# gildas-lormeau/zlib-streams-ts

Measured on AMD Instinct MI355X. Metric: uncompressed MB/s, deflate-raw L6, 4096x64KiB batch at 1/2/4/8 GPUs, higher is better.
Workload: dtype u8; 1 GPU; 4096 x 65536 B text-corpus streams split across the GPUs, deflate-raw level 6; global_streams=4096, streams_per_gpu=4096, stream_bytes=65536, level=6, format=deflate-raw, compressed_bytes=91855591, parallelism=dp1

## Files before the change

zlib-streams-ts_amd/csrc/capi.cpp:

```cpp
#include <hip/hip_runtime.h>
#include <stdint.h>
#include <stdio.h>
#include <string.h>

#include <algorithm>
#include <string>
#include <thread>
#include <type_traits>
#include <vector>

#include "../../include/zs_gpu.h"
#include "zs_common.h"
#include "zs_kernels.h"
#include "zs_inflate.h"
#include "zs_split.h"
#include "zs_seg.h"
#include "zs_plan.h"
#include "zs_dict.h"


namespace {

thread_local std::string g_err;

int fail(int code, const char* fmt, const char* a = "") {
  char buf[512];
  snprintf(buf, sizeof buf, fmt, a);
  g_err = buf;
  return code;
}

#define HIPCHK(x)                                                          \
  do {                                                                     \
    hipError_t e_ = (x);                                                   \
    if (e_ != hipSuccess) return fail(ZS_MEM_ERROR, "%s", hipGetErrorString(e_)); \
  } while (0)

template <bool kHost>
struct BufT {
  void* p = nullptr;
  size_t cap = 0;
  BufT() = default;
  BufT(const BufT&) = delete;
  BufT& operator=(const BufT&) = delete;
  ~BufT() { release(); }
  void release() {
    if (p) (void)(kHost ? hipHostFree(p) : hipFree(p));
    p = nullptr;
    cap = 0;
  }
// ... 384 lines not shown
  HIPCHK(hipGetLastError());
  return ZS_OK;
}

struct DeflDict {
  const Batch* data;
  const uint32_t *start, *did, *dadler;
};
static int deflate_launch(zs_ctx* c, hipStream_t st, int level, int wrap, const zs_level_cfg& cfg, const Batch& b,
                          const MetaLayout& ml, int32_t* d_status, uint32_t* d_out_len, const DeflDict* dd = nullptr) {
  const zs_deflate_plan& p = c->dp;
  const uint32_t n = b.n;
  const uint8_t* dm = c->meta.as<uint8_t>();
  const uint64_t* d_pos = (const uint64_t*)(dm + ml.pos_base);
  const uint32_t* d_blk = (const uint32_t*)(dm + ml.blk_base);
  const zs_sweep_seg* d_segs = (const zs_sweep_seg*)(dm + ml.segs);
  zs_stream* d_st = c->streams.as<zs_stream>();
  zs_block* d_bk = c->blocks.as<zs_block>();
  uint32_t* syms = c->syms.as<uint32_t>();
  uint32_t* check = c->check.as<uint32_t>();
  const int nthreads_s = 256, nblocks_s = (int)((n + 255) / 256);
  MARK("start");
  if (wrap) {
    const Batch& d = dd ? *dd->data : b;
    zs_k_checksum<<<n, 64, 0, st>>>(d.in, d.in_off, d.in_len, check, wrap == 1 ? 1 : 2);
    zs_k_copy_check<<<nblocks_s, nthreads_s, 0, st>>>(check, d_st, (int)n);
    MARK("checksum");
  }
  if (level >= 4 && c->o.match_sweep) {
    const uint32_t nw = (uint32_t)p.segs.size();
    (c->lane_order ? zs_k_bucket<true> : zs_k_bucket<false>)<<<nw, ZS_BK_THREADS, 0, st>>>(
        b.in, b.in_off, b.in_len, d_pos, d_segs, c->prevd.as<uint16_t>(), c->mres.as<uint2>());
    MARK("bucket");
    zs_k_sweep<<<nw, 1024, 0, st>>>(b.in, b.in_off, b.in_len, d_pos, d_segs, c->prevd.as<uint16_t>(),
                                    c->mres.as<uint2>(), cfg.chain, cfg.nice);
    MARK("sweep");
  } else if (level >= 4) {
    const dim3 g((p.max_len + 8191) / 8192, n);
    (c->lane_order ? zs_k_prev<true> : zs_k_prev<false>)<<<n, 64, 0, st>>>(b.in, b.in_off, b.in_len, d_pos,
                                                                           c->prevd.as<uint16_t>(), 0u);
    MARK("prev");
    if (p.max_len) zs_k_match<<<g, 1024, 0, st>>>(b.in, b.in_off, b.in_len, d_pos, c->prevd.as<uint16_t>(),
                                                   c->mres.as<uint2>(), cfg.chain, cfg.nice, 0u);
    MARK("match");
  }
  if (level >= 4) {
    const int pw = p.pw;
    if (dd) {
      auto parse = pw == 4 ? zs_k_parse_4w_dict : pw == 2 ? zs_k_parse_2w_dict : zs_k_parse_dict;
      parse<<<n, 64 * pw, 0, st>>>(b.in, b.in_off, b.in_len, d_pos, d_blk, c->mres.as<uint2>(), syms, d_bk, d_st,
                                   c->pscr.as<uint32_t>(), cfg.good, cfg.lazy, dd->start);
    } else {
      auto parse = pw == 4 ? zs_k_parse_4w : pw == 2 ? zs_k_parse_2w : zs_k_parse;
      parse<<<n, 64 * pw, 0, st>>>(b.in, b.in_off, b.in_len, d_pos, d_blk, c->mres.as<uint2>(), syms, d_bk, d_st,
                                   c->pscr.as<uint32_t>(), cfg.good, cfg.lazy);
    }
    MARK("parse");
  } else {
    const int fast_smem = 2 * 32768 * 2 + 32768;
    auto pick = [&](auto D) {
      constexpr bool DICT = decltype(D)::value;
      return !c->fast_group ? zs_k_fast_serial<DICT>
             : c->lane_order ? (cfg.nice <= 8 ? zs_k_fast<2, true, DICT> : cfg.nice <= 16 ? zs_k_fast<4, true, DICT> : zs_k_fast<8, true, DICT>)
                             : (cfg.nice <= 8 ? zs_k_fast<2, false, DICT> : cfg.nice <= 16 ? zs_k_fast<4, false, DICT> : zs_k_fast<8, false, DICT>);
    };
    auto fast = dd ? pick(std::true_type{}) : pick(std::false_type{});
    HIPCHK(hipFuncSetAttribute((const void*)fast, hipFuncAttributeMaxDynamicSharedMemorySize, fast_smem));
    fast<<<n, 64, fast_smem, st>>>(b.in, b.in_off, b.in_len, d_pos, d_blk, syms, d_bk, d_st, cfg.chain, cfg.lazy,
// ... 990 lines not shown
```

zlib-streams-ts_amd/csrc/deflate_sweep.hip:

```cpp
#include <hip/hip_runtime.h>
#include "zs_common.h"
#include "zs_kernels.h"
#include "zs_sweep_ring.h"
#include "zs_sweep_long.h"
#include <type_traits>

#define ZS_SW_WIN_WORDS ((ZS_SEG_WPOS + 258u + 20u + 3u) / 4u + 2u)
#define ZS_SW_RING 128u
#define ZS_SW_MW 320u
#ifndef ZS_SW_RUN_CAP
#define ZS_SW_RUN_CAP 16u
#endif

typedef __attribute__((address_space(3))) uint32_t zs_sw_lds_u32;
static __device__ __forceinline__ uint32_t sw_lds_addr(const void* p) {
  return (uint32_t)(uintptr_t)(const zs_sw_lds_u32*)p;
}

static __device__ __forceinline__ uint32_t sw_hash(uint32_t w) {
  return (((w & 0xffu) << 10) ^ (((w >> 8) & 0xffu) << 5) ^ ((w >> 16) & 0xffu)) & ZS_HASH_MASK;
}

#define ZS_BK_WPT (16384u / ZS_BK_THREADS)
#define ZS_BK_PPL (ZS_BK_THREADS / 64u)
#ifndef ZS_BK_PROF
#define ZS_BK_PROF 0
#endif
#if ZS_BK_PROF
__device__ unsigned long long zs_bk_stat[4];
extern "C" int zs_bucket_stats(unsigned long long* out) {
  return (int)hipMemcpyFromSymbol(out, HIP_SYMBOL(zs_bk_stat), sizeof(zs_bk_stat));
}
#define BK_MARK(i) do { if (threadIdx.x == 0) { const unsigned long long t_ = wall_clock64(); atomicAdd(&zs_bk_stat[i], t_ - bk_t); bk_t = t_; } } while (0)
#else
#define BK_MARK(i) do { } while (0)
#endif
#define ZS_BK_INFLIGHT 8
#define ZS_BK_CHUNK 2048u
// ... 163 lines not shown
          if (p < c1) qc[p - c0] = (uint16_t)(e[j] >> sh[j]);
        }
      }
    } else if (wave != 0 && c > 0) {
      const uint32_t b0 = c0 - ZS_BK_CHUNK, cnt1 = min(m, c0) - b0;
      const uint16_t* const qp = q[(c - 1) & 1u];
      for (uint32_t o = tid - 64u; o < cnt1; o += ZS_BK_THREADS - 64u) mem[qp[o]] = (uint16_t)(b0 + o);
    }
    __syncthreads();
  }
  BK_MARK(2);
}
template __global__ void zs_k_bucket<true>(const uint8_t*, const uint64_t*, const uint32_t*, const uint64_t*,
                                           const zs_sweep_seg*, uint16_t*, uint2*);
template __global__ void zs_k_bucket<false>(const uint8_t*, const uint64_t*, const uint32_t*, const uint64_t*,
                                            const zs_sweep_seg*, uint16_t*, uint2*);

static __device__ __forceinline__ uint32_t sw_word(const uint32_t* win, uint32_t off) {
  const uint32_t i = off >> 2;
  return __builtin_amdgcn_alignbyte(win[i + 1], win[i], off & 3u);
}

static __device__ __forceinline__ uint32_t sw_extend(const uint32_t* win, uint32_t p, uint32_t q, uint32_t maxc,
                                                     uint32_t from) {
  uint32_t k = from;
  while (k < maxc) {
    const uint32_t y = sw_word(win, q + k) ^ sw_word(win, p + k);
    if (y) { k += (uint32_t)(__builtin_ctz(y) >> 3); break; }
    k += 4;
  }
  return k < maxc ? k : maxc;
}

static __device__ __forceinline__ uint64_t sw_uniform(uint64_t x) {
  return ((uint64_t)(uint32_t)__builtin_amdgcn_readfirstlane((uint32_t)(x >> 32)) << 32) |
         (uint64_t)(uint32_t)__builtin_amdgcn_readfirstlane((uint32_t)x);
}

static __device__ __forceinline__ uint32_t max3(uint32_t a, uint32_t b, uint32_t c) {
  return max(max(a, b), c);
}

static __device__ __forceinline__ uint32_t sw_x7(uint32_t w) {
  const uint32_t b0 = w & 0xffu, b1 = (w >> 8) & 0xffu;
  return ((b0 >> 5) & 3u) | ((b1 & 7u) << 2) | (((b1 >> 5) & 3u) << 5);
}
template <bool A7>
struct SwSig;
template <>
struct SwSig<false> {
  static constexpr uint32_t LONG = 88u;
  static constexpr uint32_t THR0 = 23u;
  static constexpr uint32_t EXT = 11u;
  uint32_t a, b, c;
  static __device__ __forceinline__ uint4 rec(const uint32_t* win, uint32_t q, uint32_t w0) {
    return make_uint4(w0, sw_word(win, q + 4), sw_word(win, q + 8) & 0x00ffffffu, 0u);
  }
  __device__ __forceinline__ uint32_t mbits(uint32_t x, uint32_t y, uint32_t z) const {
    uint32_t f0, f1, f2;
    asm("v_ffbl_b32 %0, %1" : "=v"(f0) : "v"(x ^ a));
    asm("v_ffbl_b32 %0, %1\n\tv_add_u32_e64 %0, %0, 32 clamp" : "=&v"(f1) : "v"(y ^ b));
    asm("v_ffbl_b32 %0, %1\n\tv_add_u32_e32 %0, 64, %0" : "=&v"(f2) : "v"(z ^ c));
    return min(min(f0, f1), f2);
  }
  static __device__ __forceinline__ uint32_t len(uint32_t sigma) { return sigma; }
};
template <>
struct SwSig<true> {
  static constexpr uint32_t LONG = 64u;
  static constexpr uint32_t THR0 = 7u;
  static constexpr uint32_t EXT = 10u;
  uint32_t a, b;
  static __device__ __forceinline__ uint4 rec(const uint32_t* win, uint32_t q, uint32_t w0) {
    return make_uint4(sw_x7(w0) | (sw_word(win, q + 3) << 8), sw_word(win, q + 6), sw_word(win, q + EXT), 0u);
  }
  __device__ __forceinline__ uint32_t mbits(uint32_t x, uint32_t y, uint32_t) const {
    uint32_t f0, f1;
    asm("v_ffbl_b32 %0, %1" : "=v"(f0) : "v"(x ^ a));
    asm("v_ffbl_b32 %0, %1\n\tv_add_u32_e64 %0, %0, 32 clamp" : "=&v"(f1) : "v"(y ^ b));
    return min(min(f0, f1), 64u);
  }
  static __device__ __forceinline__ uint32_t len(uint32_t sigma) { return sigma ? sigma + 2u : 2u; }
};

struct SwRing {
  uint2 ab[2 * ZS_SW_RING];
  uint32_t c[2 * ZS_SW_RING];
  uint32_t key[2 * ZS_SW_RING];
  __device__ __forceinline__ void put(int b, uint32_t lane, uint4 r) {
    const uint32_t i = (uint32_t)(64 * b + (int)lane) & (ZS_SW_RING - 1);
    ab[i] = make_uint2(r.x, r.y);
    ab[i + ZS_SW_RING] = make_uint2(r.x, r.y);
    c[i] = r.z;
    c[i + ZS_SW_RING] = r.z;
    key[i] = r.w;
    key[i + ZS_SW_RING] = r.w;
  }
  static __device__ __forceinline__ uint32_t base(int c, uint32_t s, uint32_t lane) {
    return ((uint32_t)(64 * (c - (int)s - 1) + (int)lane) & (ZS_SW_RING - 1)) + 64u * s + 64u;
  }
};
struct SwRingP {
  uint2 ab[ZS_SWR_SLOTS + ZS_SWR_MIRROR];
  uint32_t c[ZS_SWR_SLOTS + ZS_SWR_MIRROR];
  uint32_t key[ZS_SWR_SLOTS + ZS_SWR_MIRROR];
  __device__ __forceinline__ void put(int b, uint32_t lane, uint4 r) {
    const uint32_t i = zs_swr_block_slot(b) + lane;
    ab[i] = make_uint2(r.x, r.y);
    c[i] = r.z;
    key[i] = r.w;
    if (zs_swr_mirrored(b)) {
      ab[i + ZS_SWR_SLOTS] = make_uint2(r.x, r.y);
      c[i + ZS_SWR_SLOTS] = r.z;
      key[i + ZS_SWR_SLOTS] = r.w;
    }
  }
  static __device__ __forceinline__ uint32_t base(int c, uint32_t s, uint32_t lane) { return zs_swr_base(c, s) + lane; }
  __device__ __forceinline__ uint32_t pos(int c, uint32_t lane, uint32_t t) const {
    return key[zs_swr_member_slot(c, lane, t)] & 0xffffu;
  }
};

#ifndef ZS_SW_PROF
#define ZS_SW_PROF 0
#endif
#if ZS_SW_PROF
__device__ unsigned long long zs_sw_stat[8];
#define SW_STAT(i, v) do { if ((threadIdx.x & 63u) == __builtin_ctzll(__builtin_amdgcn_read_exec())) atomicAdd(&zs_sw_stat[i], (unsigned long long)(v)); } while (0)
extern "C" int zs_sw_stats(unsigned long long* out) {
  return (int)hipMemcpyFromSymbol(out, HIP_SYMBOL(zs_sw_stat), sizeof(zs_sw_stat));
}
#else
#define SW_STAT(i, v) do { } while (0)
#endif

static __device__ __forceinline__ uint32_t sw_score(uint32_t mb, uint32_t u) { return (mb & ~7u) | (7u - u); }
template <uint32_t N>
static __device__ __forceinline__ uint32_t sw_gmax(const uint32_t* sc) {
  static_assert(N == 8 || N == 4 || N == 3 || N == 1, "group sizes");
  if constexpr (N == 8) return max(max3(sc[0], sc[1], sc[2]), max3(sc[3], sc[4], max3(sc[5], sc[6], sc[7])));
  else if constexpr (N == 4) return max3(sc[0], sc[1], max(sc[2], sc[3]));
  else if constexpr (N == 3) return max3(sc[0], sc[1], sc[2]);
  else return sc[0];
}

template <bool A7>
struct SwLane {
  SwSig<A7> S;
  uint32_t p;
  bool own;
  uint32_t maxc, nice;
  uint32_t khead, klim;
  uint32_t long_m;
  uint32_t own_ext;
  uint32_t thr, bt, thr_s, bt_s;
  uint32_t lthr, lbt, lthr_s, lbt_s;
  uint64_t alive_m;
  uint32_t head;
  bool snapped;
  __device__ __forceinline__ bool tail() const { return maxc <= 12u; }
  __device__ __forceinline__ void snap() {
    thr_s = thr;
    bt_s = bt;
    lthr_s = lthr;
    lbt_s = lbt;
    snapped = true;
  }
};

template <bool A7, bool MW, bool PR>
struct SwWave {
  using Sig = SwSig<A7>;
  using Lane = SwLane<A7>;
  using Ring = std::conditional_t<PR, SwRingP, SwRing>;
  const uint32_t* win;
  Ring* R;
  uint16_t* mw;
  const uint16_t* mem;
  uint32_t n, m, lane;
  uint32_t budget, budget_s, nice_cfg;
  int cc;
  zs_swr_range vr;
  int mw0;

  __device__ __forceinline__ int k() const { return 64 * cc + (int)lane; }
  __device__ __forceinline__ uint32_t fetch(int j) const { return j >= 0 && (uint32_t)j < m ? (uint32_t)mem[j] : 0u; }
  __device__ __forceinline__ uint4 make_rec(uint32_t q) const {
    const uint32_t w0 = sw_word(win, q);
    uint4 r = Sig::rec(win, q, w0);
    r.w = (sw_hash(w0) << 16) | q;
    return r;
  }
  __device__ __forceinline__ void build_blk(int blk, uint32_t q) {
    const int j = 64 * blk + (int)lane;
    const bool in = j >= 0 && (uint32_t)j < m;
    if (MW && (uint32_t)(j - mw0) < ZS_SW_MW) mw[j - mw0] = (uint16_t)q;
    R->put(blk, lane, in ? make_rec(q) : make_uint4(0, 0, 0, 0));
    if constexpr (PR) vr = zs_swr_extend(vr, blk);
  }
  __device__ __forceinline__ bool missing(int blk) const { return !PR || !zs_swr_has(vr, blk); }
  __device__ __forceinline__ uint32_t member(uint32_t t) const {
    if constexpr (PR) return R->pos(cc, lane, t);
    const int j = k() - (int)t;
// ... 9 lines not shown
    L.p = p;
    L.own = own;
    const uint32_t h = rown.w >> 16;
    const uint32_t look = n - p;
    L.maxc = look < ZS_MAX_MATCH ? look : ZS_MAX_MATCH;
    L.nice = look < nice_cfg ? look : nice_cfg;
    L.long_m = L.tail() ? 0xffffu : Sig::LONG;
    const uint32_t limit = p > ZS_MAX_DIST ? p - ZS_MAX_DIST : 0u;
    L.khead = (h << 16) | (limit > 1u ? limit : 1u);
    L.klim = (h << 16) | limit;
    L.thr = L.thr_s = Sig::THR0;
    L.bt = L.bt_s = 0;
    L.lthr = L.lthr_s = ZS_SWL_NONE;
    L.lbt = L.lbt_s = 0;
    L.alive_m = 0;
    L.head = 0;
    L.snapped = budget_s <= 1u;
    return rown;
  }

  __device__ __forceinline__ void build(uint4 rown, uint32_t p, uint32_t qb, bool have_qb) {
    mw0 = 64 * cc - (int)budget;
    if (MW) mw[k() - mw0] = (uint16_t)p;
    __builtin_amdgcn_s_waitcnt(0xc07f);
    __builtin_amdgcn_wave_barrier();
    R->put(cc, lane, rown);
    if constexpr (PR) vr = zs_swr_push(vr, cc);
    if (missing(cc - 1)) build_blk(cc - 1, have_qb ? qb : fetch(k() - 64));
    __builtin_amdgcn_s_waitcnt(0xc07f);
    __builtin_amdgcn_wave_barrier();
  }

  __device__ __forceinline__ void fold(Lane& L, uint32_t gm, uint32_t t0, const uint32_t* sc, uint32_t cnt,
                                       uint32_t base) const {
    const bool up = gm > (L.thr | 7u);
    L.thr = up ? gm : L.thr;
    L.bt = up ? t0 : L.bt;
    if (__builtin_expect(__builtin_amdgcn_ballot_w64(gm >= L.long_m) != 0, 0)) {
      SW_STAT(3, 1);
      auto lscore = [&](uint32_t u) -> uint32_t {
        const uint32_t ls = base - (t0 + u);
        const uint32_t x = (A7 ? R->c[ls] : sw_word(win, (R->key[ls] & 0xffffu) + Sig::EXT)) ^ L.own_ext;
        const uint32_t len = x ? Sig::EXT + ((uint32_t)__builtin_ctz(x) >> 3)
                               : sw_extend(win, L.p, R->key[ls] & 0xffffu, L.maxc, Sig::EXT + 4u);
        return zs_swl_score(len, L.maxc, L.nice, u);
      };
      const bool lg = gm >= L.long_m && zs_swl_open(L.lthr, L.nice);
      uint32_t w[2] = {0, 0};
#pragma unroll
      for (uint32_t u = 0; u < 8; u++)
        if (u < cnt) w[u >> 2] |= sc[u] << (8u * (u & 3u));
      constexpr uint32_t LB = (0x80u - Sig::LONG) * 0x01010101u;
      const uint32_t nl = (uint32_t)__builtin_popcount((w[0] + LB) & 0x80808080u) +
                          (uint32_t)__builtin_popcount((w[1] + LB) & 0x80808080u);
      const uint64_t twice = __builtin_amdgcn_ballot_w64(lg && nl > 1u);
      uint32_t gl = 0;
      const uint32_t u1 = zs_swl_first(gm);
      if (lg) gl = lscore(u1);
      if (__builtin_expect(twice != 0, 0)) {
        if ((twice >> lane) & 1u) {
          uint32_t lm = 0;
#pragma unroll
          for (uint32_t u = 0; u < 8; u++) lm |= (u < cnt && sc[u] >= L.long_m) ? 1u << u : 0u;
          lm &= ~(1u << u1);
          while (lm) {
            gl = zs_swl_join(gl, lscore((uint32_t)__builtin_ctz(lm)));
            lm &= lm - 1u;
          }
        }
      }
      zs_swl_fold(gl, t0, &L.lthr, &L.lbt);
    }
  }

  template <uint32_t N>
  __device__ __forceinline__ void group_fast(Lane& L, uint32_t base, uint32_t t0, bool live) const {
    const uint32_t lo = base - (t0 + (N - 1u));
    const uint2* const A = R->ab + lo;
    const uint32_t* const C = R->c + lo;
    uint32_t sc[N];
#pragma unroll
    for (uint32_t u = 0; u < N; u++) {
      const uint2 ab = A[N - 1u - u];
      sc[u] = sw_score(L.S.mbits(ab.x, ab.y, A7 ? 0u : C[N - 1u - u]), u);
    }
    fold(L, live ? sw_gmax<N>(sc) : 0u, t0, sc, N, base);
  }
  template <uint32_t N, bool HEAD>
  __device__ __forceinline__ void group_masked(Lane& L, uint32_t base, uint32_t t0) const {
    const uint32_t lo = base - (t0 + (N - 1u));
    const uint2* const A = R->ab + lo;
    const uint32_t* const C = R->c + lo;
    const uint32_t* const K = R->key + lo;
    uint32_t sc[N], key[N];
    uint2 ab[N];
#pragma unroll
    for (uint32_t u = 0; u < N; u++) {
      key[u] = K[N - 1u - u];
      ab[u] = A[N - 1u - u];
    }
    if constexpr (HEAD) {
      const bool a1 = L.own && key[0] >= L.khead;
      L.head = a1 ? 1u | ((L.p - (key[0] & 0xffffu)) == ZS_MAX_DIST ? 0x8000u : 0u) : 0u;
      L.alive_m = __builtin_amdgcn_ballot_w64(a1);
    }
    uint64_t lm = L.alive_m;
#pragma unroll
    for (uint32_t u = 0; u < N; u++) {
      if (!HEAD || u) {
        asm("v_cmp_gt_u32_e64 %0, %1, %2" : "=s"(lm) : "v"(key[u]), "v"(L.klim));
        lm &= L.alive_m;
      }
      const uint32_t v = sw_score(L.S.mbits(ab[u].x, ab[u].y, A7 ? 0u : C[N - 1u - u]), u);
      asm("v_cndmask_b32_e64 %0, 0, %1, %2" : "=v"(sc[u]) : "v"(v), "s"(lm));
    }
    L.alive_m = sw_uniform(lm);
    fold(L, sw_gmax<N>(sc), t0, sc, N, base);
  }

  __device__ __forceinline__ void run(Lane& L, uint32_t base, uint32_t ta, uint32_t tb) const {
    auto last_of = [&](uint32_t t0) __attribute__((always_inline)) {
      uint32_t t1 = t0 + 7u <= tb ? t0 + 7u : t0 + 3u;
      if (t0 <= budget_s && t1 > budget_s) t1 = budget_s;
      return t1;
    };
    if (ta > tb) return;
    uint32_t t0 = ta, t1 = last_of(ta);
    uint32_t kl = R->key[base - t1];
    while (L.alive_m) {
      const bool mine = ((L.alive_m >> lane) & 1u) != 0;
      const uint64_t last_live = __builtin_amdgcn_ballot_w64(mine && kl > L.klim);
      const uint32_t n0 = t1 + 1u, n1 = n0 <= tb ? last_of(n0) : t1;
      kl = R->key[base - n1];
      SW_STAT(last_live == L.alive_m ? 1 : 2, 1);
      SW_STAT(4, t1 - t0 + 1u);
      if (last_live == L.alive_m) {
        if (t1 - t0 == 7u) group_fast<8>(L, base, t0, mine);
        else group_fast<4>(L, base, t0, mine);
      } else {
        if (t1 - t0 == 7u) group_masked<8, false>(L, base, t0);
        else group_masked<4, false>(L, base, t0);
      }
      if (t1 == budget_s) L.snap();
      if (n0 > tb) break;
      t0 = n0;
      t1 = n1;
    }
  }

  __device__ __forceinline__ void sweep(Lane& L) {
    const uint32_t base0 = Ring::base(cc, 0u, lane);
    const bool open8 = budget_s >= 8u && budget >= 8u;
    if (open8) {
      group_masked<8, true>(L, base0, 1u);
      if (budget_s == 8u) L.snap();
    } else {
      group_masked<1, true>(L, base0, 1u);
      if (budget_s == 1u) L.snap();
      if (budget >= 4u) {
        group_masked<3, false>(L, base0, 2u);
        if (budget_s == 4u) L.snap();
      }
    }
    for (uint32_t b = 0; budget > 4u && L.alive_m; b++) {
      const int blk = cc - (int)b - 1;
      if (b >= 1 && missing(blk)) {
        __builtin_amdgcn_s_waitcnt(0xc07f);
        __builtin_amdgcn_wave_barrier();
        build_blk(blk, fetch(64 * blk + (int)lane));
        __builtin_amdgcn_s_waitcnt(0xc07f);
        __builtin_amdgcn_wave_barrier();
      }
      const uint32_t ta = b == 0 ? (open8 ? 9u : 5u) : 64u * b + 1u;
      const uint32_t tb = min(64u * b + 64u, budget);
      run(L, Ring::base(cc, b, lane), ta, tb);
      if (tb >= budget) break;
    }
    if (!L.snapped) L.snap();
  }

  __device__ __forceinline__ void settle(const Lane& L, uint2* out) const {
    __builtin_amdgcn_s_waitcnt(0xc07f);
    __builtin_amdgcn_wave_barrier();
    if (!L.own) return;
    const uint32_t p = L.p;
    uint32_t rx = 0, ry = 0;
    if (L.head) {
      uint32_t len = 2, dist = 0, len_s = 2, dist_s = 0;
      if (L.tail()) {
        const int k = this->k();
        uint32_t b = 2u << 16, bs = 2u << 16;
        for (uint32_t t = 1; t <= budget && (int)t <= k; t++) {
          const uint32_t q = member(t);
          const uint32_t key = (sw_hash(sw_word(win, q)) << 16) | q;
          if (t == 1u ? key < L.khead : key <= L.klim) break;
          uint32_t len = 12;
          for (uint32_t o = 0; o < 12u; o += 4) {
            const uint32_t y = sw_word(win, q + o) ^ sw_word(win, p + o);
            if (y) { len = o + (uint32_t)(__builtin_ctz(y) >> 3); break; }
          }
          const uint32_t sc = ((len < L.maxc ? len : L.maxc) << 16) | (0xffffu - t);
          b = max(b, sc);
          if (t <= budget_s) bs = max(bs, sc);
        }
        len = b >> 16;
        dist = len > 2u ? p - (uint32_t)mem[k - (int)(0xffffu - (b & 0xffffu))] : 0u;
        len_s = bs >> 16;
        dist_s = len_s > 2u ? p - (uint32_t)mem[k - (int)(0xffffu - (bs & 0xffffu))] : 0u;
      } else {
        const uint32_t tb = L.bt + 7u - (L.thr & 7u), tb_s = L.bt_s + 7u - (L.thr_s & 7u);
        if (L.bt) {
          len = Sig::len(L.thr >> 3);
          dist = p - member(tb);
        }
        if (L.bt_s) {
          len_s = Sig::len(L.thr_s >> 3);
          dist_s = tb_s == tb ? dist : p - member(tb_s);
        }
        auto long_of = [&](uint32_t lt, uint32_t t, uint32_t& ln, uint32_t& ds) {
          const uint32_t q = member(t);
          ln = lt >> 3;
          if (ln >= L.nice) ln = sw_extend(win, p, q, L.maxc, Sig::EXT);
          ds = p - q;
        };
        if (L.lbt) long_of(L.lthr, L.lbt, len, dist);
        if (L.lbt_s) {
          if (L.lbt_s == L.lbt) {
            len_s = len;
            dist_s = dist;
          } else {
            long_of(L.lthr_s, L.lbt_s, len_s, dist_s);
          }
        }
      }
      rx = (len << 16) | (len > 2u ? dist : 0u) | (L.head & 0x8000u);
      ry = (len_s << 16) | (len_s > 2u ? dist_s : 0u);
    }
    out[p] = make_uint2(rx, ry);
  }
};

template <bool A7, bool MW, bool PR>
static __device__ __forceinline__ void sw_body(const uint32_t* win, void* ringp, uint16_t* mw, uint32_t* next,
                                               uint32_t n, uint32_t m, uint32_t olo, uint32_t ohi,
                                               const uint16_t* mem, uint2* out, int chain, int nice_cfg) {
  using Wave = SwWave<A7, MW, PR>;
  const uint32_t lane = threadIdx.x & 63u;
  Wave W{win, (typename Wave::Ring*)ringp, mw, mem, n, m, lane, (uint32_t)chain, (uint32_t)chain >> 2,
         (uint32_t)nice_cfg, 0, zs_swr_empty(), 0};
  const uint32_t nchunks = (m + 63) / 64;
  auto claim = [&]() -> uint32_t {
    uint32_t c = 0;
    if (lane == 0) c = atomicAdd(next, 1u);
    return __builtin_amdgcn_readfirstlane(c);
  };
  auto claim_run = [&](uint32_t& c0, uint32_t& c1) {
    uint32_t a = 0, r = 0;
    if (lane == 0) {
      const uint32_t cur = __hip_atomic_load(next, __ATOMIC_RELAXED, __HIP_MEMORY_SCOPE_WORKGROUP);
      r = zs_swr_run_len(cur < nchunks ? nchunks - cur : 0u, ZS_SW_RUN_CAP);
      a = atomicAdd(next, r);
    }
    c0 = __builtin_amdgcn_readfirstlane(a);
    c1 = min(c0 + (uint32_t)__builtin_amdgcn_readfirstlane(r), nchunks);
  };
  uint32_t c, ce = 0;
  if constexpr (PR) claim_run(c, ce);
  else c = claim();
  uint32_t pf_p = W.fetch((int)(64 * c + lane)), pf_b = W.fetch((int)(64 * c + lane) - 64);
  bool fresh_n = true;
  for (;;) {
    if (c >= nchunks) break;
    const bool fresh = fresh_n;
    uint32_t cn, cen = ce;
    if constexpr (PR) {
      cn = c + 1u;
      fresh_n = cn >= ce;
      if (fresh_n) claim_run(cn, cen);
      if (fresh) W.vr = zs_swr_empty();
    } else {
      cn = claim();
    }
    W.cc = (int)c;
    const bool mem_ok = (uint32_t)W.k() < m;
    SW_STAT(0, 1);
    const uint32_t p = pf_p, qb = pf_b;
    if (cn < nchunks) {
      pf_p = W.fetch((int)(64 * cn + lane));
      if (!PR || fresh_n) pf_b = W.fetch((int)(64 * cn + lane) - 64);
    }
    c = cn;
    ce = cen;
    const bool own = mem_ok && p >= olo && p < ohi;
    if (__builtin_amdgcn_ballot_w64(own) == 0) {
      W.vr = zs_swr_empty();
      continue;
    }
    typename Wave::Lane L;
    const uint4 rown = W.start(L, p, mem_ok, own);
    W.build(rown, p, qb, fresh);
    W.sweep(L);
    W.settle(L, out);
  }
}

__global__ __launch_bounds__(1024) void zs_k_sweep(const uint8_t* __restrict__ in, const uint64_t* __restrict__ in_off,
                                                   const uint32_t* __restrict__ in_len,
                                                   const uint64_t* __restrict__ pos_base,
                                                   const zs_sweep_seg* __restrict__ segs,
                                                   const uint16_t* __restrict__ members, uint2* __restrict__ mres,
                                                   int chain, int nice_cfg) {
  constexpr uint32_t RING_BYTES = 16u * sizeof(SwRing), MWIN_BYTES = 16u * ZS_SW_MW * sizeof(uint16_t);
  static_assert(16u * sizeof(SwRingP) <= RING_BYTES + MWIN_BYTES, "the persistent rings must fit the old ones' LDS");
  __shared__ __attribute__((aligned(16))) uint8_t rmem[RING_BYTES + MWIN_BYTES];
  __shared__ __attribute__((aligned(16))) uint32_t win[ZS_SW_WIN_WORDS];
  __shared__ uint32_t next;
  const zs_sweep_seg G = segs[blockIdx.x];
  const int s = (int)G.s;
  const uint32_t n = in_len[s] - G.base;
  if (n < 3) return;
  const uint32_t m = min(n - 2, G.ohi);
  const uint8_t* src = in + in_off[s] + G.base;
  uint32_t hi = 0;
  if ((((uintptr_t)src) & 15u) == 0) {
    for (uint32_t i = threadIdx.x; 4 * i < ZS_SW_WIN_WORDS; i += 1024) {
      const uint32_t b = 16 * i;
      uint4 v;
      if (b + 16 <= n) v = ((const uint4*)src)[i];
      else {
        uint32_t t[4] = {0, 0, 0, 0};
        for (uint32_t k = 0; k < 16; k++)
          if (b + k < n) t[k >> 2] |= (uint32_t)src[b + k] << (8 * (k & 3));
        v = make_uint4(t[0], t[1], t[2], t[3]);
      }
      hi |= v.x | v.y | v.z | v.w;
      if (4 * i + 3 < ZS_SW_WIN_WORDS) *(uint4*)(win + 4 * i) = v;
      else for (uint32_t k = 0; 4 * i + k < ZS_SW_WIN_WORDS; k++) win[4 * i + k] = (&v.x)[k];
    }
  } else {
    for (uint32_t i = threadIdx.x; i < ZS_SW_WIN_WORDS; i += 1024) {
      uint32_t v = 0;
      for (uint32_t k = 0; k < 4; k++)
        if (4 * i + k < n) v |= (uint32_t)src[4 * i + k] << (8 * k);
      hi |= v;
      win[i] = v;
    }
  }
  if (threadIdx.x == 0) next = 0;
  const bool a7 = !__syncthreads_or((hi & 0x80808080u) != 0);
  const uint32_t wave = threadIdx.x >> 6;
  const uint16_t* mem = members + G.mb;
  uint2* out = mres + pos_base[s] + G.base;
  const uint32_t olo = G.olo, ohi = G.ohi;
  if (chain <= (int)ZS_SWR_MAX_CHAIN) {
    SwRingP* const R = reinterpret_cast<SwRingP*>(rmem) + wave;
    if (a7) sw_body<true, false, true>(win, R, nullptr, &next, n, m, olo, ohi, mem, out, chain, nice_cfg);
    else sw_body<false, false, true>(win, R, nullptr, &next, n, m, olo, ohi, mem, out, chain, nice_cfg);
    return;
  }
  SwRing* const R = reinterpret_cast<SwRing*>(rmem) + wave;
  uint16_t* const mw = reinterpret_cast<uint16_t*>(rmem + RING_BYTES) + wave * ZS_SW_MW;
  if (chain + 64 <= (int)ZS_SW_MW) {
    if (a7) sw_body<true, true, false>(win, R, mw, &next, n, m, olo, ohi, mem, out, chain, nice_cfg);
    else sw_body<false, true, false>(win, R, mw, &next, n, m, olo, ohi, mem, out, chain, nice_cfg);
  } else {
    if (a7) sw_body<true, false, false>(win, R, mw, &next, n, m, olo, ohi, mem, out, chain, nice_cfg);
    else sw_body<false, false, false>(win, R, mw, &next, n, m, olo, ohi, mem, out, chain, nice_cfg);
  }
}
```

zlib-streams-ts_amd/csrc/zs_kernels.h:

```cpp
#pragma once
#include <hip/hip_runtime.h>
#include <stdint.h>
#include "zs_plan.h"

struct zs_block {
  uint32_t sym_start;
  uint32_t sym_count;
  uint32_t in_start;
  uint32_t in_end;
  uint32_t type;
  uint32_t hdr_bits;
  uint32_t data_bits;
  uint32_t last;
  uint32_t pad;
  uint64_t bit_off;
  uint64_t bit_end;
};

struct zs_stream {
  uint32_t nsym;
  uint32_t nblk;
  uint64_t total_bits;
  uint32_t out_len;
  int32_t status;
  uint32_t check;
  uint32_t pad;
};

template <bool ORD>
__global__ void zs_k_prev(const uint8_t* in, const uint64_t* in_off, const uint32_t* in_len, const uint64_t* pos_base,
                          uint16_t* prevd, uint32_t min_len);
__global__ void zs_k_match(const uint8_t* in, const uint64_t* in_off, const uint32_t* in_len, const uint64_t* pos_base,
                           const uint16_t* prevd, uint2* mres, int chain, int nice, uint32_t min_len);
#define ZS_BK_THREADS 512u
template <bool ORD>
__global__ void zs_k_bucket(const uint8_t* in, const uint64_t* in_off, const uint32_t* in_len, const uint64_t* pos_base,
                            const zs_sweep_seg* segs, uint16_t* members, uint2* mres);
__global__ void zs_k_sweep(const uint8_t* in, const uint64_t* in_off, const uint32_t* in_len, const uint64_t* pos_base,
                           const zs_sweep_seg* segs, const uint16_t* members, uint2* mres, int chain, int nice);
#define ZS_PARSE_DECL(name)                                                                                        \
  __global__ void name(const uint8_t* in, const uint64_t* in_off, const uint32_t* in_len, const uint64_t* pos_base, \
                       const uint32_t* blk_base, const uint2* mres, uint32_t* syms, zs_block* blocks,              \
                       zs_stream* streams, uint32_t* scratch, int good, int lazy);                                 \
  __global__ void name##_dict(const uint8_t* in, const uint64_t* in_off, const uint32_t* in_len,                   \
                              const uint64_t* pos_base, const uint32_t* blk_base, const uint2* mres, uint32_t* syms, \
                              zs_block* blocks, zs_stream* streams, uint32_t* scratch, int good, int lazy,         \
                              const uint32_t* dstart);
ZS_PARSE_DECL(zs_k_parse)
ZS_PARSE_DECL(zs_k_parse_2w)
ZS_PARSE_DECL(zs_k_parse_4w)
template <int NW, bool ORD, bool DICT>
__global__ void zs_k_fast(const uint8_t* in, const uint64_t* in_off, const uint32_t* in_len, const uint64_t* pos_base,
                          const uint32_t* blk_base, uint32_t* syms, zs_block* blocks, zs_stream* streams, int chain,
                          int lazy, int nice, const uint32_t* dstart);
template <bool DICT>
__global__ void zs_k_fast_serial(const uint8_t* in, const uint64_t* in_off, const uint32_t* in_len,
                                 const uint64_t* pos_base, const uint32_t* blk_base, uint32_t* syms, zs_block* blocks,
                                 zs_stream* streams, int chain, int lazy, int nice, const uint32_t* dstart);
__global__ void zs_k_dict_join(const uint8_t* in, const uint64_t* in_off, const uint32_t* in_len, const uint8_t* dict,
                               const uint64_t* dict_off, const uint32_t* dict_len, const uint32_t* dstart,
                               uint8_t* joined, const uint64_t* joff);
__global__ void zs_k_trees(const uint8_t* in, const uint64_t* in_off, const uint64_t* pos_base, const uint32_t* blk_base,
                           const uint32_t* syms, zs_block* blocks, const zs_stream* streams, uint32_t* codes,
                           uint32_t* hdr, int nstreams);
__global__ void zs_k_layout(const uint32_t* blk_base, zs_block* blocks, zs_stream* streams, const uint32_t* out_cap,
                            uint8_t* out, const uint64_t* out_off, int wrap, int nstreams);
__global__ void zs_k_layout_dict(const uint32_t* blk_base, zs_block* blocks, zs_stream* streams, const uint32_t* out_cap,
                                 uint8_t* out, const uint64_t* out_off, int wrap, int nstreams, const uint32_t* dstart);
__global__ void zs_k_wrap_dict(const zs_stream* streams, uint8_t* out, const uint64_t* out_off, const uint32_t* in_len,
                               int wrap, int level, int nstreams, const uint32_t* dstart, const uint32_t* did,
// ... 13 lines not shown
```

zlib-streams-ts_amd/csrc/zs_sweep_ring.h:

```cpp
#ifndef ZS_SWEEP_RING_H
#define ZS_SWEEP_RING_H
#include <stdint.h>

#if defined(__HIPCC__)
#define ZS_SWR_FN static __host__ __device__ __forceinline__
#else
#define ZS_SWR_FN static inline
#endif

#define ZS_SWR_BLOCKS 3u
#define ZS_SWR_SLOTS 192u
#define ZS_SWR_MIRROR 64u
#define ZS_SWR_MAX_CHAIN 128u
#define ZS_SWR_RUN_DIV 32u

ZS_SWR_FN uint32_t zs_swr_block_slot(int32_t b) { return 64u * ((uint32_t)(b + 3) % ZS_SWR_BLOCKS); }

ZS_SWR_FN int zs_swr_mirrored(int32_t b) { return zs_swr_block_slot(b) == 0u; }

ZS_SWR_FN uint32_t zs_swr_base(int32_t c, uint32_t s) {
  return zs_swr_block_slot(c - (int32_t)s - 1) + 64u * s + 64u;
}

ZS_SWR_FN uint32_t zs_swr_member_slot(int32_t c, uint32_t l, uint32_t t) {
  const uint32_t s = zs_swr_block_slot(c - 2) + 128u + l - t;
  return s >= ZS_SWR_SLOTS ? s - ZS_SWR_SLOTS : s;
}

typedef struct { int32_t lo, hi; } zs_swr_range;

ZS_SWR_FN zs_swr_range zs_swr_empty(void) {
  zs_swr_range r;
  r.lo = 1;
  r.hi = 0;
  return r;
}
ZS_SWR_FN int zs_swr_has(zs_swr_range r, int32_t b) { return r.lo <= b && b <= r.hi; }

ZS_SWR_FN zs_swr_range zs_swr_push(zs_swr_range r, int32_t c) {
  if (r.lo > r.hi || r.hi != c - 1) {
    r.lo = c;
  } else if (r.lo < c - 2) {
    r.lo = c - 2;
  }
  r.hi = c;
  return r;
}
ZS_SWR_FN zs_swr_range zs_swr_extend(zs_swr_range r, int32_t b) {
  r.lo = b;
  return r;
}

ZS_SWR_FN uint32_t zs_swr_run_len(uint32_t left, uint32_t cap) {
  const uint32_t r = left / ZS_SWR_RUN_DIV;
  return r < 1u ? 1u : (r > cap ? cap : r);
}

#endif
```

Before: 20650 MB/s.

## Specialize sweep kernel for 8-aligned chain budgets with fused scoring asm

Adds a template flag selecting a sweep path when chain and its quarter are multiples of 8, processing candidate groups of exactly 8 in a tight loop that prefetches the next key and only applies per-candidate masking when a group ends the live run. Scoring is fused into a short asm sequence (xor, ffbl, min3, and_or, cndmask), and the readfirstlane uniformization of the alive mask is dropped. This aims to cut branching, group-size dispatch and VALU instructions in the match-finding inner loop, at the cost of doubling kernel instantiations and more complex hand-written asm.

```diff
diff --git a/zlib-streams-ts_amd/csrc/capi.cpp b/zlib-streams-ts_amd/csrc/capi.cpp
--- a/zlib-streams-ts_amd/csrc/capi.cpp
+++ b/zlib-streams-ts_amd/csrc/capi.cpp
@@ -16,6 +16,7 @@
 #include "zs_split.h"
 #include "zs_seg.h"
 #include "zs_plan.h"
+#include "zs_sweep_ring.h"
 #include "zs_dict.h"
 
 
@@ -466,8 +467,8 @@
     (c->lane_order ? zs_k_bucket<true> : zs_k_bucket<false>)<<<nw, ZS_BK_THREADS, 0, st>>>(
         b.in, b.in_off, b.in_len, d_pos, d_segs, c->prevd.as<uint16_t>(), c->mres.as<uint2>());
     MARK("bucket");
-    zs_k_sweep<<<nw, 1024, 0, st>>>(b.in, b.in_off, b.in_len, d_pos, d_segs, c->prevd.as<uint16_t>(),
-                                    c->mres.as<uint2>(), cfg.chain, cfg.nice);
+    (zs_sweep_uniform8(cfg.chain) ? zs_k_sweep<true> : zs_k_sweep<false>)<<<nw, 1024, 0, st>>>(
+        b.in, b.in_off, b.in_len, d_pos, d_segs, c->prevd.as<uint16_t>(), c->mres.as<uint2>(), cfg.chain, cfg.nice);
     MARK("sweep");
   } else if (level >= 4) {
     const dim3 g((p.max_len + 8191) / 8192, n);
diff --git a/zlib-streams-ts_amd/csrc/deflate_sweep.hip b/zlib-streams-ts_amd/csrc/deflate_sweep.hip
--- a/zlib-streams-ts_amd/csrc/deflate_sweep.hip
+++ b/zlib-streams-ts_amd/csrc/deflate_sweep.hip
@@ -4,6 +4,7 @@
 #include "zs_sweep_ring.h"
 #include "zs_sweep_long.h"
 #include <type_traits>
+#include <utility>
 
 #define ZS_SW_WIN_WORDS ((ZS_SEG_WPOS + 258u + 20u + 3u) / 4u + 2u)
 #define ZS_SW_RING 128u
@@ -233,11 +234,6 @@
   return k < maxc ? k : maxc;
 }
 
-static __device__ __forceinline__ uint64_t sw_uniform(uint64_t x) {
-  return ((uint64_t)(uint32_t)__builtin_amdgcn_readfirstlane((uint32_t)(x >> 32)) << 32) |
-         (uint64_t)(uint32_t)__builtin_amdgcn_readfirstlane((uint32_t)x);
-}
-
 static __device__ __forceinline__ uint32_t max3(uint32_t a, uint32_t b, uint32_t c) {
   return max(max(a, b), c);
 }
@@ -264,6 +260,16 @@
     asm("v_ffbl_b32 %0, %1\n\tv_add_u32_e32 %0, 64, %0" : "=&v"(f2) : "v"(z ^ c));
     return min(min(f0, f1), f2);
   }
+  template <uint32_t U>
+  __device__ __forceinline__ uint32_t step(uint32_t x, uint32_t y, uint32_t z) const {
+    return (mbits(x, y, z) & ~7u) | (7u - U);
+  }
+  template <uint32_t U>
+  __device__ __forceinline__ uint32_t step(uint32_t x, uint32_t y, uint32_t z, uint64_t lm) const {
+    uint32_t r;
+    asm("v_cndmask_b32_e64 %0, 0, %1, %2" : "=v"(r) : "v"(step<U>(x, y, z)), "s"(lm));
+    return r;
+  }
   static __device__ __forceinline__ uint32_t len(uint32_t sigma) { return sigma; }
 };
 template <>
@@ -280,6 +286,33 @@
     asm("v_ffbl_b32 %0, %1" : "=v"(f0) : "v"(x ^ a));
     asm("v_ffbl_b32 %0, %1\n\tv_add_u32_e64 %0, %0, 32 clamp" : "=&v"(f1) : "v"(y ^ b));
     return min(min(f0, f1), 64u);
+  }
+  template <uint32_t U>
+  __device__ __forceinline__ uint32_t step(uint32_t x, uint32_t y, uint32_t) const {
+    asm("v_xor_b32_e32 %0, %0, %2\n\t"
+        "v_xor_b32_e32 %1, %1, %3\n\t"
+        "v_ffbl_b32 %0, %0\n\t"
+        "v_ffbl_b32 %1, %1\n\t"
+        "v_add_u32_e64 %1, %1, 32 clamp\n\t"
+        "v_min3_u32 %0, %0, %1, 64\n\t"
+        "v_and_or_b32 %0, %0, -8, %4"
+        : "+v"(x), "+v"(y)
+        : "v"(a), "v"(b), "n"(7u - U));
+    return x;
+  }
+  template <uint32_t U>
+  __device__ __forceinline__ uint32_t step(uint32_t x, uint32_t y, uint32_t, uint64_t lm) const {
+    asm("v_xor_b32_e32 %0, %0, %2\n\t"
+        "v_xor_b32_e32 %1, %1, %3\n\t"
+        "v_ffbl_b32 %0, %0\n\t"
+        "v_ffbl_b32 %1, %1\n\t"
+        "v_add_u32_e64 %1, %1, 32 clamp\n\t"
+        "v_min3_u32 %0, %0, %1, 64\n\t"
+        "v_and_or_b32 %0, %0, -8, %4\n\t"
+        "v_cndmask_b32_e64 %0, 0, %0, %5"
+        : "+v"(x), "+v"(y)
+        : "v"(a), "v"(b), "n"(7u - U), "s"(lm));
+    return x;
   }
   static __device__ __forceinline__ uint32_t len(uint32_t sigma) { return sigma ? sigma + 2u : 2u; }
 };
@@ -335,7 +368,14 @@
 #define SW_STAT(i, v) do { } while (0)
 #endif
 
-static __device__ __forceinline__ uint32_t sw_score(uint32_t mb, uint32_t u) { return (mb & ~7u) | (7u - u); }
+template <class F, uint32_t... U>
+static __device__ __forceinline__ void sw_each_(F&& f, std::integer_sequence<uint32_t, U...>) {
+  (f(std::integral_constant<uint32_t, U>{}), ...);
+}
+template <uint32_t N, class F>
+static __device__ __forceinline__ void sw_each(F&& f) {
+  sw_each_(f, std::make_integer_sequence<uint32_t, N>{});
+}
 template <uint32_t N>
 static __device__ __forceinline__ uint32_t sw_gmax(const uint32_t* sc) {
   static_assert(N == 8 || N == 4 || N == 3 || N == 1, "group sizes");
@@ -369,7 +409,7 @@
   }
 };
 
-template <bool A7, bool MW, bool PR>
+template <bool A7, bool MW, bool PR, bool U8>
 struct SwWave {
   using Sig = SwSig<A7>;
   using Lane = SwLane<A7>;
@@ -445,17 +485,17 @@
   }
 
   __device__ __forceinline__ void fold(Lane& L, uint32_t gm, uint32_t t0, const uint32_t* sc, uint32_t cnt,
-                                       uint32_t base) const {
+                                       const uint32_t* gc, const uint32_t* gk) const {
     const bool up = gm > (L.thr | 7u);
     L.thr = up ? gm : L.thr;
     L.bt = up ? t0 : L.bt;
     if (__builtin_expect(__builtin_amdgcn_ballot_w64(gm >= L.long_m) != 0, 0)) {
       SW_STAT(3, 1);
       auto lscore = [&](uint32_t u) -> uint32_t {
-        const uint32_t ls = base - (t0 + u);
-        const uint32_t x = (A7 ? R->c[ls] : sw_word(win, (R->key[ls] & 0xffffu) + Sig::EXT)) ^ L.own_ext;
+        const uint32_t ls = cnt - 1u - u;
+        const uint32_t x = (A7 ? gc[ls] : sw_word(win, (gk[ls] & 0xffffu) + Sig::EXT)) ^ L.own_ext;
         const uint32_t len = x ? Sig::EXT + ((uint32_t)__builtin_ctz(x) >> 3)
-                               : sw_extend(win, L.p, R->key[ls] & 0xffffu, L.maxc, Sig::EXT + 4u);
+                               : sw_extend(win, L.p, gk[ls] & 0xffffu, L.maxc, Sig::EXT + 4u);
         return zs_swl_score(len, L.maxc, L.nice, u);
       };
       const bool lg = gm >= L.long_m && zs_swl_open(L.lthr, L.nice);
@@ -486,31 +526,38 @@
     }
   }
 
+  struct Grp {
+    const uint2* A;
+    const uint32_t *C, *K;
+  };
   template <uint32_t N>
-  __device__ __forceinline__ void group_fast(Lane& L, uint32_t base, uint32_t t0, bool live) const {
+  __device__ __forceinline__ Grp at(uint32_t base, uint32_t t0) const {
     const uint32_t lo = base - (t0 + (N - 1u));
-    const uint2* const A = R->ab + lo;
-    const uint32_t* const C = R->c + lo;
+    return Grp{R->ab + lo, R->c + lo, R->key + lo};
+  }
+  __device__ __forceinline__ const uint32_t* c_of(const Grp& g) const {
+    if constexpr (A7) return R->c + ((sw_lds_addr(g.A) - sw_lds_addr(R->ab)) >> 3);
+    else return g.C;
+  }
+  template <uint32_t N>
+  __device__ __forceinline__ void group_fast(Lane& L, const Grp& g, uint32_t t0) const {
     uint32_t sc[N];
-#pragma unroll
-    for (uint32_t u = 0; u < N; u++) {
-      const uint2 ab = A[N - 1u - u];
-      sc[u] = sw_score(L.S.mbits(ab.x, ab.y, A7 ? 0u : C[N - 1u - u]), u);
-    }
-    fold(L, live ? sw_gmax<N>(sc) : 0u, t0, sc, N, base);
+    sw_each<N>([&](auto uc) __attribute__((always_inline)) {
+      constexpr uint32_t u = decltype(uc)::value;
+      const uint2 ab = g.A[N - 1u - u];
+      sc[u] = L.S.template step<u>(ab.x, ab.y, A7 ? 0u : g.C[N - 1u - u]);
+    });
+    const uint32_t gm = __builtin_amdgcn_inverse_ballot_w64(L.alive_m) ? sw_gmax<N>(sc) : 0u;
+    fold(L, gm, t0, sc, N, c_of(g), g.K);
   }
   template <uint32_t N, bool HEAD>
-  __device__ __forceinline__ void group_masked(Lane& L, uint32_t base, uint32_t t0) const {
-    const uint32_t lo = base - (t0 + (N - 1u));
-    const uint2* const A = R->ab + lo;
-    const uint32_t* const C = R->c + lo;
-    const uint32_t* const K = R->key + lo;
+  __device__ __forceinline__ void group_masked(Lane& L, const Grp& g, uint32_t t0) const {
     uint32_t sc[N], key[N];
     uint2 ab[N];
 #pragma unroll
     for (uint32_t u = 0; u < N; u++) {
-      key[u] = K[N - 1u - u];
-      ab[u] = A[N - 1u - u];
+      key[u] = g.K[N - 1u - u];
+      ab[u] = g.A[N - 1u - u];
     }
     if constexpr (HEAD) {
       const bool a1 = L.own && key[0] >= L.khead;
@@ -518,17 +565,18 @@
       L.alive_m = __builtin_amdgcn_ballot_w64(a1);
     }
     uint64_t lm = L.alive_m;
-#pragma unroll
-    for (uint32_t u = 0; u < N; u++) {
+    sw_each<N>([&](auto uc) __attribute__((always_inline)) {
+      constexpr uint32_t u = decltype(uc)::value;
       if (!HEAD || u) {
-        asm("v_cmp_gt_u32_e64 %0, %1, %2" : "=s"(lm) : "v"(key[u]), "v"(L.klim));
-        lm &= L.alive_m;
-      }
-      const uint32_t v = sw_score(L.S.mbits(ab[u].x, ab[u].y, A7 ? 0u : C[N - 1u - u]), u);
-      asm("v_cndmask_b32_e64 %0, 0, %1, %2" : "=v"(sc[u]) : "v"(v), "s"(lm));
-    }
-    L.alive_m = sw_uniform(lm);
-    fold(L, sw_gmax<N>(sc), t0, sc, N, base);
+        uint64_t gt;
+        const uint32_t ku = key[u], klim = L.klim;
+        asm("v_cmp_gt_u32_e64 %0, %1, %2" : "=s"(gt) : "v"(ku), "v"(klim));
+        lm = gt & L.alive_m;
+      }
+      sc[u] = L.S.template step<u>(ab[u].x, ab[u].y, A7 ? 0u : g.C[N - 1u - u], lm);
+    });
+    L.alive_m = lm;
+    fold(L, sw_gmax<N>(sc), t0, sc, N, c_of(g), g.K);
   }
 
   __device__ __forceinline__ void run(Lane& L, uint32_t base, uint32_t ta, uint32_t tb) const {
@@ -541,18 +589,17 @@
     uint32_t t0 = ta, t1 = last_of(ta);
     uint32_t kl = R->key[base - t1];
     while (L.alive_m) {
-      const bool mine = ((L.alive_m >> lane) & 1u) != 0;
-      const uint64_t last_live = __builtin_amdgcn_ballot_w64(mine && kl > L.klim);
+      const uint64_t last_live = __builtin_amdgcn_ballot_w64(kl > L.klim) & L.alive_m;
       const uint32_t n0 = t1 + 1u, n1 = n0 <= tb ? last_of(n0) : t1;
       kl = R->key[base - n1];
       SW_STAT(last_live == L.alive_m ? 1 : 2, 1);
       SW_STAT(4, t1 - t0 + 1u);
       if (last_live == L.alive_m) {
-        if (t1 - t0 == 7u) group_fast<8>(L, base, t0, mine);
-        else group_fast<4>(L, base, t0, mine);
+        if (t1 - t0 == 7u) group_fast<8>(L, at<8>(base, t0), t0);
+        else group_fast<4>(L, at<4>(base, t0), t0);
       } else {
-        if (t1 - t0 == 7u) group_masked<8, false>(L, base, t0);
-        else group_masked<4, false>(L, base, t0);
+        if (t1 - t0 == 7u) group_masked<8, false>(L, at<8>(base, t0), t0);
+        else group_masked<4, false>(L, at<4>(base, t0), t0);
       }
       if (t1 == budget_s) L.snap();
       if (n0 > tb) break;
@@ -561,17 +608,67 @@
     }
   }
 
+  __device__ __forceinline__ void run8(Lane& L, uint32_t base, uint32_t ta, uint32_t te) const {
+    asm("" : "+s"(L.alive_m));
+    Grp g = at<8>(base, ta);
+    const zs_sw_lds_u32* k8 = (const zs_sw_lds_u32*)(g.K - 8);
+    uint32_t kl = g.K[0];
+    if (!L.alive_m) return;
+    uint32_t t0 = ta;
+    do {
+      const uint64_t last_live = __builtin_amdgcn_ballot_w64(kl > L.klim) & L.alive_m;
+      kl = k8[0];
+      g.K = (const uint32_t*)(k8 + 8);
+      SW_STAT(last_live == L.alive_m ? 1 : 2, 1);
+      SW_STAT(4, 8u);
+      const uint64_t a0 = L.alive_m;
+      const bool ends = last_live != a0;
+      uint32_t sc[8], key[8];
+      if (ends) {
+#pragma unroll
+        for (uint32_t u = 0; u < 8; u++) key[u] = g.K[7u - u];
+      }
+      sw_each<8>([&](auto uc) __attribute__((always_inline)) {
+        constexpr uint32_t u = decltype(uc)::value;
+        const uint2 ab = g.A[7u - u];
+        sc[u] = L.S.template step<u>(ab.x, ab.y, A7 ? 0u : g.C[7u - u]);
+      });
+      if (ends) {
+        uint64_t lm = a0;
+        sw_each<8>([&](auto uc) __attribute__((always_inline)) {
+          constexpr uint32_t u = decltype(uc)::value;
+          uint64_t gt;
+          const uint32_t ku = key[u], klim = L.klim;
+          asm("v_cmp_gt_u32_e64 %0, %1, %2" : "=s"(gt) : "v"(ku), "v"(klim));
+          lm = gt & a0;
+          const uint64_t lmu = lm;
+          uint32_t v = sc[u];
+          asm("v_cndmask_b32_e64 %0, 0, %0, %1" : "+v"(v) : "s"(lmu));
+          sc[u] = v;
+        });
+        L.alive_m = lm;
+      }
+      const uint32_t gm = __builtin_amdgcn_inverse_ballot_w64(a0) ? sw_gmax<8>(sc) : 0u;
+      fold(L, gm, t0, sc, 8u, c_of(g), g.K);
+      t0 += 8u;
+      g.A -= 8;
+      if (!A7) g.C -= 8;
+      k8 -= 8;
+      asm("" : "+v"(k8));
+    } while (t0 <= te && L.alive_m);
+  }
+
   __device__ __forceinline__ void sweep(Lane& L) {
     const uint32_t base0 = Ring::base(cc, 0u, lane);
-    const bool open8 = budget_s >= 8u && budget >= 8u;
+    const bool open8 = U8 || (budget_s >= 8u && budget >= 8u);
     if (open8) {
-      group_masked<8, true>(L, base0, 1u);
+      group_masked<8, true>(L, at<8>(base0, 1u), 1u);
       if (budget_s == 8u) L.snap();
-    } else {
-      group_masked<1, true>(L, base0, 1u);
+    } else if constexpr (!U8) {
+      group_masked<1, true>(L, at<1>(base0, 1u), 1u);
       if (budget_s == 1u) L.snap();
       if (budget >= 4u) {
-        group_masked<3, false>(L, base0, 2u);
+        group_masked<3, false>(L, at<3>(base0, 2u), 2u);
         if (budget_s == 4u) L.snap();
       }
     }
@@ -584,9 +681,20 @@
         __builtin_amdgcn_s_waitcnt(0xc07f);
         __builtin_amdgcn_wave_barrier();
       }
-      const uint32_t ta = b == 0 ? (open8 ? 9u : 5u) : 64u * b + 1u;
+      uint32_t ta = b == 0 ? (open8 ? 9u : 5u) : 64u * b + 1u;
       const uint32_t tb = min(64u * b + 64u, budget);
-      run(L, Ring::base(cc, b, lane), ta, tb);
+      const uint32_t base = Ring::base(cc, b, lane);
+      if constexpr (U8) {
+        while (ta <= tb && L.alive_m) {
+          const bool cut = !L.snapped && budget_s <= tb;
+          const uint32_t te = cut ? budget_s : tb;
+          run8(L, base, ta, te);
+          if (cut) L.snap();
+          ta = te + 1u;
+        }
+      } else {
+        run(L, base, ta, tb);
+      }
       if (tb >= budget) break;
     }
     if (!L.snapped) L.snap();
@@ -653,11 +761,11 @@
   }
 };
 
-template <bool A7, bool MW, bool PR>
+template <bool A7, bool MW, bool PR, bool U8>
 static __device__ __forceinline__ void sw_body(const uint32_t* win, void* ringp, uint16_t* mw, uint32_t* next,
                                                uint32_t n, uint32_t m, uint32_t olo, uint32_t ohi,
                                                const uint16_t* mem, uint2* out, int chain, int nice_cfg) {
-  using Wave = SwWave<A7, MW, PR>;
+  using Wave = SwWave<A7, MW, PR, U8>;
   const uint32_t lane = threadIdx.x & 63u;
   Wave W{win, (typename Wave::Ring*)ringp, mw, mem, n, m, lane, (uint32_t)chain, (uint32_t)chain >> 2,
          (uint32_t)nice_cfg, 0, zs_swr_empty(), 0};
@@ -717,6 +825,7 @@
   }
 }
 
+template <bool U8>
 __global__ __launch_bounds__(1024) void zs_k_sweep(const uint8_t* __restrict__ in, const uint64_t* __restrict__ in_off,
                                                    const uint32_t* __restrict__ in_len,
                                                    const uint64_t* __restrict__ pos_base,
@@ -767,17 +876,21 @@
   const uint32_t olo = G.olo, ohi = G.ohi;
   if (chain <= (int)ZS_SWR_MAX_CHAIN) {
     SwRingP* const R = reinterpret_cast<SwRingP*>(rmem) + wave;
-    if (a7) sw_body<true, false, true>(win, R, nullptr, &next, n, m, olo, ohi, mem, out, chain, nice_cfg);
-    else sw_body<false, false, true>(win, R, nullptr, &next, n, m, olo, ohi, mem, out, chain, nice_cfg);
+    if (a7) sw_body<true, false, true, U8>(win, R, nullptr, &next, n, m, olo, ohi, mem, out, chain, nice_cfg);
+    else sw_body<false, false, true, U8>(win, R, nullptr, &next, n, m, olo, ohi, mem, out, chain, nice_cfg);
     return;
   }
   SwRing* const R = reinterpret_cast<SwRing*>(rmem) + wave;
   uint16_t* const mw = reinterpret_cast<uint16_t*>(rmem + RING_BYTES) + wave * ZS_SW_MW;
   if (chain + 64 <= (int)ZS_SW_MW) {
-    if (a7) sw_body<true, true, false>(win, R, mw, &next, n, m, olo, ohi, mem, out, chain, nice_cfg);
-    else sw_body<false, true, false>(win, R, mw, &next, n, m, olo, ohi, mem, out, chain, nice_cfg);
+    if (a7) sw_body<true, true, false, U8>(win, R, mw, &next, n, m, olo, ohi, mem, out, chain, nice_cfg);
+    else sw_body<false, true, false, U8>(win, R, mw, &next, n, m, olo, ohi, mem, out, chain, nice_cfg);
   } else {
-    if (a7) sw_body<true, false, false>(win, R, mw, &next, n, m, olo, ohi, mem, out, chain, nice_cfg);
-    else sw_body<false, false, false>(win, R, mw, &next, n, m, olo, ohi, mem, out, chain, nice_cfg);
-  }
-}
+    if (a7) sw_body<true, false, false, U8>(win, R, mw, &next, n, m, olo, ohi, mem, out, chain, nice_cfg);
+    else sw_body<false, false, false, U8>(win, R, mw, &next, n, m, olo, ohi, mem, out, chain, nice_cfg);
+  }
+}
+template __global__ void zs_k_sweep<true>(const uint8_t*, const uint64_t*, const uint32_t*, const uint64_t*,
+                                          const zs_sweep_seg*, const uint16_t*, uint2*, int, int);
+template __global__ void zs_k_sweep<false>(const uint8_t*, const uint64_t*, const uint32_t*, const uint64_t*,
+                                           const zs_sweep_seg*, const uint16_t*, uint2*, int, int);
diff --git a/zlib-streams-ts_amd/csrc/zs_kernels.h b/zlib-streams-ts_amd/csrc/zs_kernels.h
--- a/zlib-streams-ts_amd/csrc/zs_kernels.h
+++ b/zlib-streams-ts_amd/csrc/zs_kernels.h
@@ -36,6 +36,7 @@
 template <bool ORD>
 __global__ void zs_k_bucket(const uint8_t* in, const uint64_t* in_off, const uint32_t* in_len, const uint64_t* pos_base,
                             const zs_sweep_seg* segs, uint16_t* members, uint2* mres);
+template <bool U8>
 __global__ void zs_k_sweep(const uint8_t* in, const uint64_t* in_off, const uint32_t* in_len, const uint64_t* pos_base,
                            const zs_sweep_seg* segs, const uint16_t* members, uint2* mres, int chain, int nice);
 #define ZS_PARSE_DECL(name)                                                                                        \
diff --git a/zlib-streams-ts_amd/csrc/zs_sweep_ring.h b/zlib-streams-ts_amd/csrc/zs_sweep_ring.h
--- a/zlib-streams-ts_amd/csrc/zs_sweep_ring.h
+++ b/zlib-streams-ts_amd/csrc/zs_sweep_ring.h
@@ -56,4 +56,8 @@
   return r < 1u ? 1u : (r > cap ? cap : r);
 }
 
+ZS_SWR_FN int zs_sweep_uniform8(int32_t chain) {
+  return chain >= 8 && chain % 8 == 0 && (chain >> 2) >= 8 && (chain >> 2) % 8 == 0;
+}
+
 #endif
```

New measurement: 21620 MB/s (median of 6 runs). 4.7% higher.
